# johnnyjana730/MVIN

Measured on AMD Instinct MI355X. Metric: (user,item) pairs scored/sec @ dim=64 hop=2 fan-out=32; % HBM roofline, higher is better.
Workload: dtype f32

## Files before the change

mvin_amd/csrc/mvin_kernels.h:

```cpp
#pragma once
#include <hip/hip_runtime.h>
#include <stdint.h>

#include "../../include/mvin_hip.h"
#include "mvin_common.h"

namespace mvin {

struct GatherAttnArgs {
    int gather;
    int table_bf16;
    const void* table;
    const int32_t* adj_e;
    const int32_t* adj_r;
    const int32_t* node_ids;
    const float* neigh;
    const int32_t* rel_ids;
    const float* rel_score;
    const float* self_vec;
    const float* Wc;
    const float* c_child;
    const float* Wagg;
    const float* bagg;
    float* out;
    float* probs;
    float* s_out;
    float* z_out;
    int64_t T;
    int N, K, D, lpr_log2;
    int tile_rows;
};

struct RippleArgs {
    const void* E;
    int table_bf16;
    const int32_t* score_ids;
    const int32_t* rel_ids;
    const int32_t* value_ids;
    const float* V;
    const float* w;
    float* out;
    int64_t ldo;
    int64_t B;
    int mode, Nm, D, nR, lpr_log2;
};

struct RippleBuildArgs {
    const int64_t* indptr;
    const int32_t* dst;
    const int32_t* rel;
    const int64_t* hist_ptr;
    const int32_t* hist_items;
    int32_t* out;
    int64_t n_user;
    uint64_t seed;
    int P, Nm, n_neighbor;
};

struct KeyAddrArgs {
    const void* E;
    const float* V;
    const float* w;
    const int32_t* mem_h[8];
    const int32_t* mem_r[8];
    const int32_t* mem_t[8];
    float* out;
    int64_t ldo;
    int64_t B;
    int P, Nm, D, nR, lpr_log2;
    uint64_t table_bytes;
    const int32_t* uts;
    const int64_t* users64;
    const int32_t* users32;
    int n_user;
    int n_entity;
};

struct KeyAddrLists {
    const int32_t *h, *r, *t;
};
__device__ __forceinline__ KeyAddrLists key_addr_lists(const KeyAddrArgs& a, int64_t b, int hop) {
    if (a.uts) {
        int64_t u = a.users64 ? a.users64[b] : (int64_t)a.users32[b];
        u = u < 0 ? 0 : (u >= a.n_user ? a.n_user - 1 : u);
        const int32_t* base = a.uts + ((u * (a.P > 0 ? a.P : 1) + hop) * 3) * (int64_t)a.Nm;
        return {base, base + a.Nm, base + 2 * a.Nm};
    }
    const int64_t o = b * a.Nm;
    return {a.mem_h[hop] + o, hop < a.P ? a.mem_r[hop] + o : nullptr, hop < a.P ? a.mem_t[hop] + o : nullptr};
}

struct KeyAddrGroupedArgs {
    const void* E;
    const float* R;
    const float* w;
    const int32_t* uts;
    const int32_t* seg_user;
    const int32_t* seg_ptr;
    const int32_t* nseg_dev;
    const int32_t* pair_index;
    const int64_t* items64;
    const int32_t* items32;
    float* out;
    int64_t ldo;
    int nseg, P, Nm, D, nR, NRL;
    int n_entity;
    int dbg;
    const int32_t* records;
    const float* ER;
    const float* hs;
};

struct KaFlashArgs {
    const float* E;
    const float* ER;
    const float* hs;
    const int32_t* records;
    const int32_t* seg_user;
    const int32_t* seg_ptr;
    const int32_t* nseg_dev;
    const int32_t* pair_index;
    const int64_t* items64;
    const int32_t* items32;
    const float* TW;
    const float* bmlp;
    float* user_o;
    int32_t* slot_seg;
    int32_t* counter;
    int nslots;
    int P, Nm, nR, n_entity;
    int64_t B;
};

struct KaRecLayout {
    int NmP, rows, maxtiles, o_cnt, o_off, o_trel, o_bidx, o_head, o_tail, o_hr, len;
};

struct TailArgs {
    const void* E;
    const int64_t* items64;
    const int32_t* items32;
    const float* q;
    const float* user_o;
    const float* nagg0;
    const float* nagg1;
    const float* W0;
    const float* b0;
    const float* A0;
    const float* a0;
    const float* A1;
    const float* a1;
    const float* Wmix;
    const float* bmix;
    float* item_emb;
    float* scores;
    float* sig;
    int64_t B;
    int table_bf16;
    int n_entity;
    int dbg;
};

struct EntityAggArgs {
    const float* tabS;
    const float* tabG;
    const float* selfS;
    const float* selfG;
    const int32_t* adj_e;
    const int32_t* adj_r;
    const float* t0;
    float* outS;
    float* outG;
    int n_entity, K, nR;
    uint64_t table_bytes, adj_bytes;
    int D;
};

struct TailFoldArgs {
    const float* M0;
    const int64_t* items64;
    const int32_t* items32;
    const float* q;
    const float* user_o;
    const float* out0;
    const float* z2;
    const float* Wqm;
    const float* A1;
    const float* a1;
    const float* Wmix;
    const float* bm;
    float* item_emb;
    float* scores;
    float* sig;
    int64_t B;
    int n_entity;
};

struct GatherMixArgs {
    const void* table;
    const int32_t* adj_e;
    const int32_t* adj_r;
    const int32_t* node_ids;
    const float* rel_score;
    const float* rowbias;
    float* out;
    int64_t nodes;
    int npg, K, D, lpr_log2, relu, table_bf16;
};

struct FusedL2Args {
    const void* table;
    const int32_t* adj_e;
    const int32_t* adj_r;
    const int32_t* parent_ids;
    const float* t0;
    const float* t1;
    const float* W1;
    const float* W2;
    const float* q;
    const float* b1;
    const float* b2;
    const float* A0;
    const float* a0;
    float* nagg0;
    float* nagg1;
    float* probs_parent;
    float* probs_child;
    int64_t P;
    uint64_t table_bytes;
    uint64_t adj_bytes;
    int parents_per_pair, K, nR, lpn_log2;
    int pid_stride;
    unsigned max_id;
    int dbg;
    const int32_t* order;
    float* agg;
    int fold;
    int prj;
};

__device__ __forceinline__ int fused_parent_id(const FusedL2Args& a, int64_t i) {
    const unsigned v = (unsigned)a.parent_ids[i * a.pid_stride];
    return (int)(v < a.max_id ? v : a.max_id);
}

struct EltArgs {
    int mode;
    int64_t n;
    float* x;
    float* y;
    float* z;
    float* w;
    float* accum;
    float alpha, beta, beta1, beta2, eps;
    int D, N;
};

struct WgradArgs {
    mvin_linear_args lin;
    const float* dY;
    int64_t ldy, dy_zstride;
    const float* mask;
    int64_t ldm, mask_zstride;
    float* dW;
    int64_t dw_zstride;
    float* db;
    int64_t db_zstride;
    int IB;
};

struct AggBwdArgs {
    int gather;
    const float* table;
    const int32_t* adj_e;
    const int32_t* adj_r;
    const int32_t* node_ids;
    const float* child;
    const int32_t* rel_ids;
    const float* probs;
    const float* rel_score;
    int skip_zero;
    const float* dvec;
    float* dtable;
    float* dchild;
    float* dT;
    int64_t T;
    int K, D, nR, lpr_log2;
};

struct KeyAddrBwdArgs {
    KeyAddrArgs f;
    const float* dout;
    float* dE;
    float* dV;
    float* dw;
    float l2;
    const float* Rk;
    const void* items;
    int items64;
    int dw_rep;
    int dv_lds;
    float* reg_accum;
};

hipError_t launch_eltwise(const EltArgs& a, hipStream_t st);
hipError_t launch_l2_adam_multi(const mvin_param_seg* segs, int nseg, int64_t total, float* g, float* mo, float* vo,
                                float* accum, int apply_adam, float lr_t, const float* lr_dev, float b1, float b2,
                                float eps, hipStream_t st);
hipError_t launch_l2_adam_multi_guarded(const mvin_param_seg* segs, int nseg, int64_t total, float* g, float* mo, float* vo,
                                        float* accum, int apply_adam, const mvin_guard_state* guard, float b1, float b2,
                                        float eps, hipStream_t st);
hipError_t launch_grad_guard(const mvin_param_seg* segs, int nseg, int64_t total, const float* g,
                             const mvin_guard_item* items, int nitems, mvin_guard_partial* partials,
                             const float* lr_table, int lr_table_len, mvin_guard_state* state, int grid_cap,
                             hipStream_t st);
hipError_t launch_scatter_add_rows(float* dtable, const int32_t* ids, int ids64, const float* x, int64_t rows, int D,
                                   float alpha, hipStream_t st);
hipError_t launch_linear_wgrad(WgradArgs a, hipStream_t st);
hipError_t launch_linear_wgrad_multi(const WgradArgs* probs, int n, hipStream_t st);
hipError_t launch_agg_bwd(const AggBwdArgs& a, hipStream_t st);
hipError_t launch_rel_score_bwd(const float* rel, const float* urh_w, const float* dT, int nR, int D, float* drel,
                                float* durh, hipStream_t st);
hipError_t launch_key_addr_bwd(const KeyAddrBwdArgs& a, hipStream_t st);

inline int lpr_log2_for(int D) {
    int l = 0;
    while ((4 << l) < D) ++l;
    return l;
}

hipError_t launch_expand(const int32_t* adj_e, const int32_t* adj_r, const int64_t* items64,
                         const int32_t* items32, int B, int K, int levels, int n_entity,
                         int32_t* ent_out, int32_t* rel_out, hipStream_t st);
hipError_t launch_rel_score(const float* rel, const float* urh_w, int nR, int D, float* t,
                            hipStream_t st);
hipError_t launch_linear(const mvin_linear_args& a, hipStream_t st);
bool linear_mfma_supported(const mvin_linear_args& a);
hipError_t launch_linear_mfma(const mvin_linear_args& a, hipStream_t st);
hipError_t launch_gather_attn(const GatherAttnArgs& a, hipStream_t st);
hipError_t launch_ripple(const RippleArgs& a, hipStream_t st);
hipError_t launch_sample_adjacency(const int64_t* indptr, const int32_t* dst, const int32_t* rel, int n_entity,
                                   int K, uint64_t seed, int32_t* adj_e, int32_t* adj_r, hipStream_t st);
hipError_t launch_ripple_build(const RippleBuildArgs& a, hipStream_t st);
int key_addr_nj(int Nm, int D);
bool key_addr_grouped_supported(int D, int P, int Nm, int nR);
hipError_t launch_key_addr_grouped(const KeyAddrGroupedArgs& a, int table_bf16, hipStream_t st);
bool key_addr_wave16_supported(int D, int P, int Nm, int nR);
bool key_addr_wave16_applies(const KeyAddrGroupedArgs& a);
hipError_t launch_key_addr_wave16(const KeyAddrGroupedArgs& a, int table_bf16, hipStream_t st);
bool key_addr_dense_supported(int D, int P, int Nm, int nR);
hipError_t launch_key_addr_dense(const KeyAddrGroupedArgs& a, int table_bf16, hipStream_t st);
KaRecLayout ka_rec_layout(int P, int Nm, int nR);
hipError_t launch_user_records(const int32_t* uts, int n_user, int P, int Nm, int nR, int n_entity, int32_t* out, hipStream_t st);
bool key_addr_static_supported(int D, int P, int Nm, int nR);
bool key_addr_static_applies(const KeyAddrGroupedArgs& a, int table_bf16);
hipError_t launch_key_addr_static(const KeyAddrGroupedArgs& a, hipStream_t st);
bool key_addr_flash_supported(int D, int P, int Nm, int nR, int n_entity);
size_t key_addr_flash_ws_elems(int64_t B, int nseg_bound);
hipError_t launch_key_addr_flash(const KaFlashArgs& a, int nseg_bound, bool has_set, int32_t* sched_ws, hipStream_t st);
hipError_t kas_read_trace(long long* host_dst, size_t n);
hipError_t kaf_read_trace(long long* host_dst, size_t n);
hipError_t fold_read_trace(long long* host_dst, size_t n);
hipError_t launch_key_addr(const KeyAddrArgs& a, int table_bf16, hipStream_t st);
bool key_addr_stream_supported(const KeyAddrArgs& a, int table_bf16);
hipError_t launch_key_addr_stream(const KeyAddrArgs& a, int table_bf16, hipStream_t st);
hipError_t launch_move_rows(void* table, const int32_t* ids, int64_t n, int row_bytes, void* rows, bool scatter,
                            hipStream_t st);
hipError_t launch_shard_space_ids(const void* ids, bool is64, int64_t n, int world, int n_local, void* out, hipStream_t st);
hipError_t launch_row_softmax(const float* x, int64_t rows, int n, float* out, hipStream_t st);
hipError_t launch_mix_urv(const float* neigh, const float* rel, const float* user, const float* logits, int64_t nodes, int N, int K,
                          int D, float* out, float* probs, hipStream_t st);
hipError_t launch_gather_mix(const GatherMixArgs& a, hipStream_t st);
struct ScoreSmallArgs {
    const void* E;
    const int32_t* adj_e;
    const int32_t* adj_r;
    const float* R;
    const float* w_h;
    const float* Wu;
    const float* bu;
    const float* t0;
    const float* t1;
    const float *W0, *b0, *W1, *b1, *W2, *b2;
    const float *A0, *a0, *A1, *a1, *Wmix, *bmix;
    const int64_t* items;
    const int32_t* mem_h[4];
    const int32_t* mem_r[4];
    const int32_t* mem_t[4];
    const int32_t* uts;
    const int64_t* users;
    float* user_o;
    float* item_emb;
    float* scores;
    float* sig;
    int64_t B;
    int G;
    int K, P, Nm, nR, n_entity, n_user, enc, table_bf16;
    int depth1;
    int dbg;
    uint64_t table_bytes;
    uint64_t adj_bytes;
};
bool score_small_supported(int D, int K, int P, int Nm, int nR);
int score_small_group(int D, int K, int P, int Nm, int nR, int has_hset, int64_t B);
hipError_t launch_score_small(ScoreSmallArgs a, int D, hipStream_t st);
hipError_t small_read_trace(long long* host_dst, size_t n);

bool l2_tail_supported(int D);
hipError_t launch_l2_tail(const TailArgs& a, int D, hipStream_t st);
bool l2_tail_flash_applies(const TailArgs& a, int D);
hipError_t launch_l2_tail_flash(const TailArgs& a, hipStream_t st);
bool fused_l2_supported(int D, int K);
hipError_t launch_gather_attn_l2(const FusedL2Args& a, int D, int table_bf16, hipStream_t st);
bool fused_split_supported(int D, int K);
bool fused_split_applies(const FusedL2Args& a, int D);
hipError_t launch_gather_probe_l2(const void* table, const int32_t* ids1, const int32_t* ids2, int64_t n_parents, int K,
                                  int D, int table_bf16, float* sums, hipStream_t st);
hipError_t launch_group_pairs(const int64_t* u64, const int32_t* u32, int64_t B, int n_user, int32_t* count, int32_t* offs,
                              int32_t* rank, int32_t* seg_user, int32_t* seg_ptr, int32_t* nseg, int32_t* pair_index, hipStream_t st);
hipError_t launch_count_ids(const int32_t* ids, int64_t n, int nbins, float* out, hipStream_t st);
bool fused_d32_supported(int D, int K);
bool fused_d32_applies(const FusedL2Args& a, int D);
bool topk_rows_supported(int k);
hipError_t launch_topk_rows(const float* scores, int64_t rows, int64_t n, int64_t ld, const int32_t* cand_ids, int64_t col_offset,
                            const int64_t* excl_ptr, const int32_t* excl_ids, const int32_t* carry_ids, const float* carry_vals, int k,
                            int32_t* out_ids, float* out_vals, hipStream_t st);
hipError_t launch_rank_positives(const float* scores, int64_t rows, int64_t n, int64_t ld, const int32_t* cand_ids, int64_t col_offset,
                                 const int64_t* excl_ptr, const int32_t* excl_ids, const int64_t* pos_ptr, const int32_t* pos_ids,
                                 int32_t* out_counts, float* out_vals, int32_t* out_eligible, hipStream_t st);
int64_t ctr_counts_ws_bytes(int64_t n_seg, int64_t seg_len);
hipError_t launch_ctr_counts(const float* scores, const int32_t* labels, int64_t n_seg, int64_t seg_len, int64_t ld, void* ws,
                             int64_t* out, hipStream_t st);
bool sample_negatives_supported(int n_item);
hipError_t launch_sample_negatives(const int64_t* excl_ptr, const int32_t* excl_ids, const int32_t* counts, const int64_t* out_ptr,
                                   int n_user, int n_item, const uint32_t* alias_tab, const uint32_t* mask_bits, uint64_t seed,
                                   uint64_t round, int32_t* out, int64_t* status,
                                   hipStream_t st);
hipError_t launch_rank_head(const float* user_o, const float* item_emb, const float* valid, int64_t n_groups, int G, int D, int mode,
                            float scale, float* scores, float* dscore, float* du, float* di, float* loss_accum, int64_t* counts,
                            hipStream_t st);
hipError_t launch_select_negatives(const float* scores, const int64_t* items, const float* valid, const int64_t* group_key,
                                   int64_t n_groups, int Gp, int n_neg, int shortlist, uint64_t seed, uint64_t round,
                                   int64_t* out_items, float* out_valid, float* out_scores, int64_t* counts,
                                   hipStream_t st);
int64_t kg_explore_ws_bytes(int n_entity, int64_t M);
hipError_t launch_kg_field(const int64_t* eptr, const int32_t* edst, const int32_t* erel, int n_entity, int64_t M,
                           const int32_t* seeds, int64_t n_seed, int hops, void* ws, uint32_t* field_bits, int64_t* out_counts,
                           hipStream_t st);
hipError_t launch_kg_explore(const int64_t* eptr, const int32_t* edst, const int32_t* erel, int n_entity, int64_t M,
                             const int32_t* adj_entity, const int32_t* adj_relation, int K, const int32_t* seeds, int64_t n_seed,
                             int hops, void* ws, uint32_t* explored_bits, int64_t* out_counts, hipStream_t st);
size_t order_ws_elems(int64_t B);
hipError_t launch_order_by_key(const int64_t* k64, const int32_t* k32, int64_t B, int32_t* ws, int32_t* order, hipStream_t st);
bool fused_wpp_supported(int D, int K);
bool fused_wpp_applies(const FusedL2Args& a, int D);
hipError_t launch_gather_attn_l2_wpp(const FusedL2Args& a, hipStream_t st);
bool fused_agg_supported(int D, int K);
bool fused_fold_supported(int D, int K);
size_t fused_fold_lds_bytes(int D, int nR, int K);
bool fused_agg_applies(const FusedL2Args& a, int D);
hipError_t launch_entity_aggregates(const EntityAggArgs& a, hipStream_t st);
hipError_t launch_fold_prepare(const float* W0, const float* b0, const float* W1, const float* b1, const float* W2, const float* b2, const float* A0,
                               const float* a0, const float* Wmix, const float* bmix, const float* A1, float c, int D, float* blk, hipStream_t st);
hipError_t launch_l2_tail_fold(const TailFoldArgs& a, hipStream_t st);
hipError_t launch_score_l2_folded(const float* agg, const float* M0, const int32_t* adj_e, const int32_t* adj_r, const int32_t* items, int pid_stride,
                                  const float* t1, const float* q, const float* user_o, const float* Wq, const float* bq, const float* Wv,
                                  const float* bv, const float* Wqm, const float* A1, const float* a1, const float* Wm1, const float* Wm2,
                                  const float* bm, float* item_emb, float* scores, float* sig, int64_t B, int K, int D, int nR, int n_entity,
                                  hipStream_t st);
hipError_t launch_gather_attn_l2_agg(const FusedL2Args& a, hipStream_t st);
hipError_t launch_gather_attn_l2_d32(const FusedL2Args& a, int table_bf16, hipStream_t st, bool encoded = false);
bool fused_d16_supported(int D, int K);
bool fused_d16_applies(const FusedL2Args& a, int D);
hipError_t launch_gather_attn_l2_d16(const FusedL2Args& a, int table_bf16, hipStream_t st);
bool fused_l2_split_in_use();
hipError_t launch_gather_attn_l2_split(const FusedL2Args& a, int D, int table_bf16, hipStream_t st);
hipError_t split_read_trace(long long* host_dst, size_t n);
bool fused_packed_supported(int D, int K);
bool key_addr_static_er_ok(int P, int Nm, int nR, int n_entity, bool has_set);
hipError_t launch_transpose_blocks(const float* R, int nR, int D, float* RT, hipStream_t st);
constexpr int kEtMaxJobs = 24;
struct EntityTableJob {
    const float* W;
    float* out;
    int w_nk;
};
hipError_t launch_entity_tables(const float* E, int n_entity, const EntityTableJob* jobs, int njobs, hipStream_t st);
hipError_t launch_entity_dot(const float* E, const float* w, int n, int D, float* out, hipStream_t st);
hipError_t launch_prj_prepare(const float* W1, const float* W2, const float* b1, const float* b2, const float* A0, const float* a0,
                              float c, int D, float* blk, hipStream_t st);
bool fused_packed_applies(const FusedL2Args& a, int D);
hipError_t pack_read_prof(long long* host_dst, size_t n);
hipError_t launch_gather_attn_l2_packed(const FusedL2Args& a, int D, int table_bf16, hipStream_t st);
hipError_t launch_encode_adjacency(const int32_t* adj_e, const int32_t* adj_r, int n_entity, int K, int32_t* cnt,
                                   int32_t* enc_e, int32_t* enc_r, hipStream_t st);
hipError_t ka_read_trace(long long* host_dst, size_t n);

}
```

mvin_amd/csrc/mvin_keyaddr_flash.hip:

```cpp
#include <cstdlib>
#include <type_traits>

#include "mvin_kernels.h"

namespace mvin {

typedef float f32x4 __attribute__((ext_vector_type(4)));

constexpr int kFlashChunk = 64;
constexpr int kFlashWaves = 4;

__global__ void ka_flash_slots_kernel(const int32_t* __restrict__ seg_ptr, const int32_t* __restrict__ nseg_dev, int nseg_bound,
                                      int32_t* __restrict__ slot_seg) {
    const int nseg = nseg_dev ? min(*nseg_dev, nseg_bound) : nseg_bound;
    for (int s = blockIdx.x * blockDim.x + threadIdx.x; s < nseg; s += gridDim.x * blockDim.x) {
        const int p0 = seg_ptr[s], p1 = seg_ptr[s + 1];
        const int first = p0 / kFlashChunk + s;
        const int nch = (p1 - p0 + kFlashChunk - 1) / kFlashChunk;
        for (int c = 0; c < nch; ++c) slot_seg[first + c] = s;
    }
}

#define KAF_FENCE() __builtin_amdgcn_sched_barrier(0)

__device__ float g_kaf_no_bias[64];
__device__ long long g_kaf_trace[64 * 16];

extern __shared__ __attribute__((aligned(16))) int32_t sKafRec[];

template <int NMT, bool HAS_SET, bool PF, bool TRACE = false>
__global__ __launch_bounds__(kFlashWaves * 64, 2) void key_addr_flash_kernel(KaFlashArgs a, KaRecLayout RL) {
    constexpr int D = 64;
    __shared__ f32x4 sUo0[kFlashWaves][4][64];
    const int lane = threadIdx.x & 63, l16 = lane & 15, q16 = lane >> 4;
    f32x4 (*myUo0)[64] = sUo0[threadIdx.x >> 6];
    const int P = a.P, NmP = RL.NmP;
    const unsigned emax = (unsigned)(a.n_entity - 1);
    const float* __restrict__ E = a.E;
    const float* __restrict__ bias = a.bmlp;
    const size_t tw_stride = (size_t)a.n_entity * D;

    struct Rows {
        float4 v[NMT][4];
    };
    auto issue_u = [&](int mt, const int (&hr)[NMT], Rows& R) {
        const f32x4* src = reinterpret_cast<const f32x4*>(a.ER + (size_t)(unsigned)max(hr[mt], 0) * D) + q16;
#pragma unroll
        for (int nt = 0; nt < 4; ++nt) {
            const f32x4 v = src[4 * nt];
            R.v[mt][nt] = make_float4(v[0], v[1], v[2], v[3]);
        }
    };
    auto issue_t = [&](int mt, const float* __restrict__ tab, const int4 (&ids)[NMT], Rows& R) {
        const int id[4] = {ids[mt].x, ids[mt].y, ids[mt].z, ids[mt].w};
#pragma unroll
        for (int i = 0; i < 4; ++i)
            R.v[mt][i] = reinterpret_cast<const float4*>(tab + (size_t)(unsigned)max(id[i], 0) * D)[l16];
    };
    auto reads_tile = [&](bool two, int mt, const Rows& R, const f32x4 (&p0)[NMT], const f32x4 (&p1)[NMT], f32x4 (&u0)[4], f32x4 (&u1)[4]) {
        if (two) {
#pragma unroll
            for (int i = 0; i < 4; ++i) {
                const float t[4] = {R.v[mt][i].x, R.v[mt][i].y, R.v[mt][i].z, R.v[mt][i].w};
#pragma unroll
                for (int nt = 0; nt < 4; ++nt) u0[nt] = __builtin_amdgcn_mfma_f32_16x16x4f32(t[nt], p0[mt][i], u0[nt], 0, 0, 0);
#pragma unroll
                for (int nt = 0; nt < 4; ++nt) u1[nt] = __builtin_amdgcn_mfma_f32_16x16x4f32(t[nt], p1[mt][i], u1[nt], 0, 0, 0);
            }
        } else {
#pragma unroll
            for (int i = 0; i < 4; ++i) {
                const float t[4] = {R.v[mt][i].x, R.v[mt][i].y, R.v[mt][i].z, R.v[mt][i].w};
#pragma unroll
                for (int nt = 0; nt < 4; ++nt) u0[nt] = __builtin_amdgcn_mfma_f32_16x16x4f32(t[nt], p0[mt][i], u0[nt], 0, 0, 0);
            }
        }
    };
    auto softmax = [&](f32x4 (&lg)[NMT], const int4 (&ids)[NMT]) {
        float mx = -INFINITY;
#pragma unroll
        for (int mt = 0; mt < NMT; ++mt) {
            const int id[4] = {ids[mt].x, ids[mt].y, ids[mt].z, ids[mt].w};
#pragma unroll
            for (int i = 0; i < 4; ++i) mx = fmaxf(mx, id[i] >= 0 ? lg[mt][i] : -INFINITY);
        }
        mx = xor32_max(xor16_max(mx));
        float z = 0.f;
#pragma unroll
        for (int mt = 0; mt < NMT; ++mt) {
            const int id[4] = {ids[mt].x, ids[mt].y, ids[mt].z, ids[mt].w};
#pragma unroll
            for (int i = 0; i < 4; ++i) {
                const float x = lean_exp(fminf(lg[mt][i] - mx, 0.f));
                const float e = id[i] >= 0 ? x : 0.f;
                lg[mt][i] = e;
                z += e;
            }
        }
        z = xor32_sum(xor16_sum(z));
        const float inv = 1.f / z;
#pragma unroll
        for (int mt = 0; mt < NMT; ++mt) {
#pragma unroll
            for (int i = 0; i < 4; ++i) lg[mt][i] *= inv;
        }
    };

    int iter = 0;
    auto stamp = [&](int slot) {
        if constexpr (TRACE) {
            if (blockIdx.x == 0 && threadIdx.x == 0 && iter >= 2 && iter < 66) g_kaf_trace[(iter - 2) * 16 + slot] = __builtin_readcyclecounter();
        }
    };
    auto load_item_raw = [&](const int (&orig)[2], unsigned (&item)[2]) {
#pragma unroll
        for (int rt = 0; rt < 2; ++rt)
            item[rt] = a.items64 ? reinterpret_cast<const unsigned*>(a.items64)[2 * (int64_t)orig[rt]] : (unsigned)a.items32[orig[rt]];
    };
    auto load_item = [&](const int (&orig)[2], unsigned (&item)[2]) {
        load_item_raw(orig, item);
#pragma unroll
        for (int rt = 0; rt < 2; ++rt) item[rt] = min(item[rt], emax);
    };

    const int wave = __builtin_amdgcn_readfirstlane((int)(threadIdx.x >> 6));
    const int stride = (int)gridDim.x * kFlashWaves;
    const int recW = (1 + 2 * P) * NmP, ldsT = NmP, ldsHr = NmP + P * NmP;
    const unsigned lds0 = (unsigned)(size_t)(__attribute__((address_space(3))) char*)sKafRec + (unsigned)(wave * 2 * recW * 4);
    const int lorig = kFlashWaves * 2 * recW + wave * 32;
    const unsigned ldsOrig = (unsigned)(size_t)(__attribute__((address_space(3))) char*)sKafRec + (unsigned)(lorig * 4);
    auto la_slots_issue = [&](long long base) -> int {
        const long long kc = base + (long long)stride * (lane + 1);
        return kc < a.nslots ? a.slot_seg[kc] : -1;
    };
    auto la_slots_take = [&](long long base, int sv, int& kN, int& sN) -> bool {
        for (;;) {
            const unsigned long long live = __ballot(sv >= 0);
            if (live) {
                const int j = __ffsll(live) - 1;
                kN = __builtin_amdgcn_readfirstlane((int)(base + (long long)stride * (j + 1)));
                sN = __builtin_amdgcn_readlane(sv, j);
                return true;
            }
            base += 64ll * stride;
            if (base + stride >= a.nslots) return false;
            sv = la_slots_issue(base);
        }
    };
    auto la_seg_issue = [&](int s) -> int {
        const int32_t* src = lane == 0 ? a.seg_user + s : a.seg_ptr + s + (lane - 1);
        return lane < 3 ? *src : 0;
    };
    auto la_seg_take = [&](int v, int k, int s, int& u, int& cbeg, int& cend) {
        u = __builtin_amdgcn_readlane(v, 0);
        const int p0 = __builtin_amdgcn_readlane(v, 1), p1 = __builtin_amdgcn_readlane(v, 2);
        cbeg = p0 + (k - (p0 / kFlashChunk + s)) * kFlashChunk;
        cend = min(p1, cbeg + kFlashChunk);
    };
    auto la_rec_issue = [&](int u, int cbeg, int cend, int par) {
        const char* src = reinterpret_cast<const char*>(a.records + (size_t)u * RL.len);
        const unsigned dst = lds0 + (unsigned)(par * recW * 4);
        for (int j0 = 0; j0 < recW; j0 += 64) {
            const int i = j0 + lane;
            if (i < recW) {
                const int voff = 4 * (i < NmP ? RL.o_head + i : RL.o_tail + (i - NmP));
                unsigned keep;
                asm volatile("s_nop 4\n\ts_mov_b32 %0, m0\n\ts_mov_b32 m0, %3\n\ts_nop 0\n\tglobal_load_lds_dword %1, %2\n\ts_mov_b32 m0, %0"
                             : "=&s"(keep)
                             : "v"(voff), "s"(src), "s"(dst + 4u * (unsigned)j0)
                             : "memory");
            }
        }
        if (lane < 32) {
            const int voff = 4 * min(lane, cend - 1 - cbeg);
            unsigned keep;
            asm volatile("s_nop 4\n\ts_mov_b32 %0, m0\n\ts_mov_b32 m0, %3\n\ts_nop 0\n\tglobal_load_lds_dword %1, %2\n\ts_mov_b32 m0, %0"
                         : "=&s"(keep)
                         : "v"(voff), "s"(a.pair_index + cbeg), "s"(ldsOrig)
                         : "memory");
        }
    };
    auto la_orig = [&](int (&orig)[2]) {
#pragma unroll
        for (int rt = 0; rt < 2; ++rt) orig[rt] = sKafRec[lorig + 16 * rt + l16];
    };
    bool nHave = false;
    int nK = 0, nS = 0, nU = 0, nCbeg = 0, nCend = 0;
    int par = 0;
    int laSlots = 0, laSeg = 0;
    unsigned itemP[2] = {0, 0};
    if constexpr (PF) {
        const long long base = (long long)((int)blockIdx.x * kFlashWaves + wave) - stride;
        nHave = la_slots_take(base, la_slots_issue(base), nK, nS);
        if (nHave) {
            la_seg_take(la_seg_issue(nS), nK, nS, nU, nCbeg, nCend);
            la_rec_issue(nU, nCbeg, nCend, par);
            asm volatile("s_waitcnt vmcnt(0)" ::: "memory");
            int o[2];
            la_orig(o);
            load_item_raw(o, itemP);
        }
    }
    for (;; ++iter) {
        stamp(0);
        int k = 0, u = 0, cbeg = 0, cend = 0;
        if constexpr (PF) {
            if (!nHave) break;
            k = nK, u = nU, cbeg = nCbeg, cend = nCend;
            asm volatile("s_waitcnt vmcnt(0)" ::: "memory");
        } else {
            if (lane == 0) k = atomicAdd(a.counter, 1) + 1;
            k = __builtin_amdgcn_readfirstlane(k);
            if (k >= a.nslots) break;
            const int s = __builtin_amdgcn_readfirstlane(a.slot_seg[k]);
            if (s < 0) continue;
            u = __builtin_amdgcn_readfirstlane(a.seg_user[s]);
            const int p0 = __builtin_amdgcn_readfirstlane(a.seg_ptr[s]), p1 = __builtin_amdgcn_readfirstlane(a.seg_ptr[s + 1]);
            cbeg = p0 + (k - (p0 / kFlashChunk + s)) * kFlashChunk;
            cend = min(p1, cbeg + kFlashChunk);
        }
        const int32_t* __restrict__ rec = a.records + (size_t)u * RL.len;
        const int lrec = (wave * 2 + par) * recW;
        stamp(1);
        auto load_hr = [&](int hop, int (&hr)[NMT]) {
#pragma unroll
            for (int mt = 0; mt < NMT; ++mt) {
                if constexpr (PF) hr[mt] = sKafRec[lrec + ldsHr + hop * NmP + 16 * mt + l16];
                else hr[mt] = rec[RL.o_hr + hop * NmP + 16 * mt + l16];
            }
        };
        auto load_tid = [&](int hop, int4 (&tid)[NMT]) {
#pragma unroll
            for (int mt = 0; mt < NMT; ++mt) {
                if constexpr (PF) tid[mt] = *reinterpret_cast<const int4*>(&sKafRec[lrec + ldsT + hop * NmP + 16 * mt + 4 * q16]);
                else tid[mt] = *reinterpret_cast<const int4*>(rec + RL.o_tail + hop * NmP + 16 * mt + 4 * q16);
            }
        };
        auto la_step_slots = [&]() {
            nHave = la_slots_take(k, laSlots, nK, nS);
            if (nHave) laSeg = la_seg_issue(nS);
        };
        auto la_step_seg = [&]() {
            if (nHave) {
                la_seg_take(laSeg, nK, nS, nU, nCbeg, nCend);
                la_rec_issue(nU, nCbeg, nCend, par ^ 1);
            }
        };
        auto la_step_items = [&](bool rows_since) {
            if (nHave) {
                if (!rows_since) asm volatile("s_waitcnt vmcnt(0)" ::: "memory");
                int o[2];
                la_orig(o);
                load_item_raw(o, itemP);
            }
        };
        auto load_orig = [&](int t0, int (&orig)[2], bool (&valid)[2]) {
#pragma unroll
            for (int rt = 0; rt < 2; ++rt) {
                const int p = t0 + 16 * rt + l16;
                valid[rt] = p < cend;
                orig[rt] = a.pair_index[min(p, cend - 1)];
            }
        };
        auto load_be = [&](const unsigned (&item)[2], float4 (&bE)[2][4]) {
#pragma unroll
            for (int rt = 0; rt < 2; ++rt) {
#pragma unroll
                for (int nt = 0; nt < 4; ++nt) bE[rt][nt] = reinterpret_cast<const float4*>(E + (size_t)item[rt] * D)[4 * nt + q16];
            }
        };

        int orig[2], origN[2];
        bool valid[2], validN[2];
        unsigned item[2];
        float4 bE[2][4];
        int hrC[NMT], hrN[NMT];
        int4 tidC[NMT];
        Rows R;
        if constexpr (PF) {
#pragma unroll
            for (int rt = 0; rt < 2; ++rt) item[rt] = min(itemP[rt], emax), valid[rt] = cbeg + 16 * rt + l16 < cend;
            la_orig(orig);
        } else {
            load_orig(cbeg, orig, valid);
        }
        load_hr(0, hrC);
        load_tid(0, tidC);
        load_orig(cbeg + 32, origN, validN);
        f32x4 uo0[4];
#pragma unroll
        for (int r = 0; r < 4; ++r) {
            const float4 b = reinterpret_cast<const float4*>(bias)[4 * q16 + r];
            uo0[0][r] = b.x, uo0[1][r] = b.y, uo0[2][r] = b.z, uo0[3][r] = b.w;
        }
        if constexpr (HAS_SET) {
            int4 hid[NMT];
            f32x4 ph[NMT];
#pragma unroll
            for (int mt = 0; mt < NMT; ++mt) {
                if constexpr (PF) hid[mt] = *reinterpret_cast<const int4*>(&sKafRec[lrec + 16 * mt + 4 * q16]);
                else hid[mt] = *reinterpret_cast<const int4*>(rec + RL.o_head + 16 * mt + 4 * q16);
            }
#pragma unroll
            for (int mt = 0; mt < NMT; ++mt) issue_t(mt, a.TW, hid, R);
            KAF_FENCE();
            stamp(11);
            if constexpr (PF) laSlots = la_slots_issue(k);
#pragma unroll
            for (int mt = 0; mt < NMT; ++mt) {
                const int id[4] = {hid[mt].x, hid[mt].y, hid[mt].z, hid[mt].w};
#pragma unroll
                for (int i = 0; i < 4; ++i) ph[mt][i] = a.hs[max(id[i], 0)];
            }
            if constexpr (!PF) load_item(orig, item);
            KAF_FENCE();
            stamp(12);
            if constexpr (PF) {
                la_step_slots();
                KAF_FENCE();
            }
            softmax(ph, hid);
            KAF_FENCE();
            stamp(13);
            f32x4 unused[4];
#pragma unroll
            for (int mt = 0; mt < NMT; ++mt) {
                reads_tile(false, mt, R, ph, ph, uo0, unused);
                KAF_FENCE();
                issue_u(mt, hrC, R);
                KAF_FENCE();
            }
            stamp(14);
        } else {
            if constexpr (!PF) load_item(orig, item);
#pragma unroll
            for (int mt = 0; mt < NMT; ++mt) issue_u(mt, hrC, R);
            if constexpr (PF) laSlots = la_slots_issue(k);
        }
        load_be(item, bE);
        if constexpr (PF && !HAS_SET) {
            KAF_FENCE();
            la_step_slots();
        }
#pragma unroll
        for (int nt = 0; nt < 4; ++nt) myUo0[nt][lane] = uo0[nt];
        KAF_FENCE();
        stamp(2);

        const int ntile = (cend - cbeg + 31) >> 5;
        int t0 = cbeg;
        int stage = 0;
        const int stage_items = min(2, 2 * ntile * P - 1);
        auto la_stage = [&]() {
            if constexpr (PF) {
                if (stage == 0) la_step_seg();
                if (stage == stage_items) la_step_items(stage_items == 2);
                ++stage;
                KAF_FENCE();
            }
        };
        auto run_tile = [&](const bool two, const bool more) {
            f32x4 uo[2][4];
#pragma unroll
            for (int rt = 0; rt < 2; ++rt) {
#pragma unroll
                for (int nt = 0; nt < 4; ++nt) uo[rt][nt] = myUo0[nt][lane];
            }
            unsigned itemN[2];
            if (more) load_item(origN, itemN);
            for (int hop = 0; hop < P; ++hop) {
                const bool last_hop = hop + 1 == P;
                const bool next_stage = !last_hop || more;
                const int hopN = last_hop ? 0 : hop + 1;
                const float* __restrict__ tw = a.TW + (size_t)(hop + (HAS_SET ? 1 : 0)) * tw_stride;
                if (next_stage) load_hr(hopN, hrN);
                KAF_FENCE();
                if (t0 == cbeg && hop < 3) stamp(3 + 4 * hop);
                f32x4 lg[2][NMT];
#pragma unroll
                for (int mt = 0; mt < NMT; ++mt) {
                    lg[0][mt] = f32x4{0.f, 0.f, 0.f, 0.f};
                    lg[1][mt] = f32x4{0.f, 0.f, 0.f, 0.f};
                    if (two) {
#pragma unroll
                        for (int nt = 0; nt < 4; ++nt) {
                            const float av[4] = {R.v[mt][nt].x, R.v[mt][nt].y, R.v[mt][nt].z, R.v[mt][nt].w};
                            const float e0[4] = {bE[0][nt].x, bE[0][nt].y, bE[0][nt].z, bE[0][nt].w};
                            const float e1[4] = {bE[1][nt].x, bE[1][nt].y, bE[1][nt].z, bE[1][nt].w};
#pragma unroll
                            for (int i = 0; i < 4; ++i) {
                                lg[0][mt] = __builtin_amdgcn_mfma_f32_16x16x4f32(av[i], e0[i], lg[0][mt], 0, 0, 0);
                                lg[1][mt] = __builtin_amdgcn_mfma_f32_16x16x4f32(av[i], e1[i], lg[1][mt], 0, 0, 0);
                            }
                        }
                    } else {
#pragma unroll
                        for (int nt = 0; nt < 4; ++nt) {
                            const float av[4] = {R.v[mt][nt].x, R.v[mt][nt].y, R.v[mt][nt].z, R.v[mt][nt].w};
                            const float e0[4] = {bE[0][nt].x, bE[0][nt].y, bE[0][nt].z, bE[0][nt].w};
#pragma unroll
                            for (int i = 0; i < 4; ++i) lg[0][mt] = __builtin_amdgcn_mfma_f32_16x16x4f32(av[i], e0[i], lg[0][mt], 0, 0, 0);
                        }
                    }
                    KAF_FENCE();
                    issue_t(mt, tw, tidC, R);
                    KAF_FENCE();
                }
                if (last_hop && more) load_be(itemN, bE);
                KAF_FENCE();
                if (t0 == cbeg && hop < 3) stamp(4 + 4 * hop);
                la_stage();
                softmax(lg[0], tidC);
                if (two) softmax(lg[1], tidC);
                KAF_FENCE();
                if (t0 == cbeg && hop < 3) stamp(5 + 4 * hop);
#pragma unroll
                for (int mt = 0; mt < NMT; ++mt) {
                    reads_tile(two, mt, R, lg[0], lg[1], uo[0], uo[1]);
                    KAF_FENCE();
                    if (next_stage) issue_u(mt, hrN, R);
                    KAF_FENCE();
                }
                if (next_stage) load_tid(hopN, tidC);
                if (t0 == cbeg && hop < 3) stamp(6 + 4 * hop);
                la_stage();
            }
#pragma unroll
            for (int rt = 0; rt < 2; ++rt) {
                if (valid[rt] && (rt == 0 || two)) {
#pragma unroll
                    for (int r = 0; r < 4; ++r)
                        *reinterpret_cast<float4*>(a.user_o + (size_t)orig[rt] * D + 16 * q16 + 4 * r) =
                            make_float4(uo[rt][0][r], uo[rt][1][r], uo[rt][2][r], uo[rt][3][r]);
                }
            }
        };
        for (int tile = 0; tile < ntile; ++tile, t0 += 32) {
            const bool more = tile + 1 < ntile;
            run_tile(cend - t0 > 16, more);
#pragma unroll
            for (int rt = 0; rt < 2; ++rt) orig[rt] = origN[rt], valid[rt] = validN[rt];
        }
        stamp(15);
        par ^= 1;
    }
}

hipError_t kaf_read_trace(long long* host_dst, size_t n) {
    const size_t have = sizeof(g_kaf_trace) / sizeof(long long);
    return hipMemcpyFromSymbol(host_dst, HIP_SYMBOL(g_kaf_trace), (n < have ? n : have) * sizeof(long long));
}
#undef KAF_FENCE

bool key_addr_flash_supported(int D, int P, int Nm, int nR, int n_entity) {
    if (D != 64 || P < 1 || P > 8 || Nm < 1 || Nm > 64) return false;
    const KaRecLayout RL = ka_rec_layout(P, Nm, nR);
    if (RL.len == 0) return false;
    return (long long)nR * n_entity < (1ll << 31);
}

size_t key_addr_flash_ws_elems(int64_t B, int nseg_bound) { return (size_t)(B / kFlashChunk + nseg_bound + 1) + 1; }

static int env_int(const char* name, int dflt) {
    const char* v = getenv(name);
    return v && *v ? atoi(v) : dflt;
}

template <int NMT>
static hipError_t launch_flash_n(const KaFlashArgs& a, const KaRecLayout& RL, bool has_set, hipStream_t st) {
    static const bool prefetch = env_int("MVIN_KAF_PREFETCH", 1) != 0;
    static const int grid_cap = env_int("MVIN_KAF_GRID", 0);
    auto k = prefetch ? (has_set ? key_addr_flash_kernel<NMT, true, true> : key_addr_flash_kernel<NMT, false, true>)
                      : (has_set ? key_addr_flash_kernel<NMT, true, false> : key_addr_flash_kernel<NMT, false, false>);
    if constexpr (NMT == 4) {
        static const bool trace = getenv("MVIN_KAF_TRACE") != nullptr;
        if (trace && has_set) k = prefetch ? key_addr_flash_kernel<4, true, true, true> : key_addr_flash_kernel<4, true, false, true>;
    }
    const size_t lds = prefetch ? (size_t)kFlashWaves * (2 * (1 + 2 * a.P) * RL.NmP + 32) * sizeof(int32_t) : 0;
    static thread_local int per_cu[2][9] = {};
    int& pc = per_cu[has_set ? 1 : 0][a.P];
    if (pc == 0) {
        int v = 0;
        if (hipOccupancyMaxActiveBlocksPerMultiprocessor(&v, reinterpret_cast<const void*>(k), kFlashWaves * 64, lds) != hipSuccess || v < 1) v = 2;
        pc = v > 8 ? 8 : v;
    }
    const int64_t want = ((int64_t)a.nslots + kFlashWaves - 1) / kFlashWaves;
    int grid = (int)(want < 256 * (int64_t)pc ? want : 256 * (int64_t)pc);
    if (grid_cap > 0 && grid > grid_cap) grid = grid_cap;
    k<<<grid, kFlashWaves * 64, lds, st>>>(a, RL);
    return hipGetLastError();
}

hipError_t launch_key_addr_flash(const KaFlashArgs& a_, int nseg_bound, bool has_set, int32_t* sched_ws, hipStream_t st) {
    KaFlashArgs a = a_;
    const KaRecLayout RL = ka_rec_layout(a.P, a.Nm, a.nR);
    if (RL.len == 0 || !sched_ws) return hipErrorInvalidValue;
    if (!a.bmlp) {
        void* zeros = nullptr;
        if (hipError_t e = hipGetSymbolAddress(&zeros, HIP_SYMBOL(g_kaf_no_bias)); e != hipSuccess) return e;
        a.bmlp = static_cast<const float*>(zeros);
    }
    a.nslots = (int)(a.B / kFlashChunk + nseg_bound + 1);
    a.slot_seg = sched_ws;
    a.counter = sched_ws + a.nslots;
    hipError_t e = hipMemsetAsync(sched_ws, 0xFF, ((size_t)a.nslots + 1) * sizeof(int32_t), st);
    if (e != hipSuccess) return e;
    {
        const int blocks = nseg_bound < 256 * 64 ? (nseg_bound + 255) / 256 : 64;
        ka_flash_slots_kernel<<<blocks > 0 ? blocks : 1, 256, 0, st>>>(a.seg_ptr, a.nseg_dev, nseg_bound, sched_ws);
        e = hipGetLastError();
        if (e != hipSuccess) return e;
    }
    switch (RL.NmP / 16) {
        case 1: return launch_flash_n<1>(a, RL, has_set, st);
        case 2: return launch_flash_n<2>(a, RL, has_set, st);
        case 3: return launch_flash_n<3>(a, RL, has_set, st);
        case 4: return launch_flash_n<4>(a, RL, has_set, st);
        default: return hipErrorInvalidValue;
    }
}

}
```

Measured before the change: 550.4 million.

## Replace sparse slot map with compacted live-chunk list for flash scheduling

The slots kernel now builds a dense list of live (segment, chunk-start) entries with a wave prefix scan and an atomic append. The old version wrote a sparse slot→segment map that waves had to scan with ballots to skip empty slots. The flash kernel walks this compacted list with a static stride by default, with an optional dynamic atomic-ticket mode behind an env var. This removes the large 0xFF memset and the empty-slot skipping, at the cost of an extra atomic pass. Per-wave trace instrumentation is also added.

```diff
diff --git a/mvin_amd/csrc/mvin_kernels.h b/mvin_amd/csrc/mvin_kernels.h
--- a/mvin_amd/csrc/mvin_kernels.h
+++ b/mvin_amd/csrc/mvin_kernels.h
@@ -125,7 +125,7 @@
     const float* TW;
     const float* bmlp;
     float* user_o;
-    int32_t* slot_seg;
+    const int32_t* live;
     int32_t* counter;
     int nslots;
     int P, Nm, nR, n_entity;
diff --git a/mvin_amd/csrc/mvin_keyaddr_flash.hip b/mvin_amd/csrc/mvin_keyaddr_flash.hip
--- a/mvin_amd/csrc/mvin_keyaddr_flash.hip
+++ b/mvin_amd/csrc/mvin_keyaddr_flash.hip
@@ -9,15 +9,32 @@
 
 constexpr int kFlashChunk = 64;
 constexpr int kFlashWaves = 4;
-
-__global__ void ka_flash_slots_kernel(const int32_t* __restrict__ seg_ptr, const int32_t* __restrict__ nseg_dev, int nseg_bound,
-                                      int32_t* __restrict__ slot_seg) {
+constexpr bool kFlashDrawDynamicDefault = false;
+
+__global__ void ka_flash_slots_kernel(const int32_t* __restrict__ seg_ptr, const int32_t* __restrict__ nseg_dev, int nseg_bound, int cap,
+                                      int32_t* __restrict__ live) {
     const int nseg = nseg_dev ? min(*nseg_dev, nseg_bound) : nseg_bound;
-    for (int s = blockIdx.x * blockDim.x + threadIdx.x; s < nseg; s += gridDim.x * blockDim.x) {
-        const int p0 = seg_ptr[s], p1 = seg_ptr[s + 1];
-        const int first = p0 / kFlashChunk + s;
-        const int nch = (p1 - p0 + kFlashChunk - 1) / kFlashChunk;
-        for (int c = 0; c < nch; ++c) slot_seg[first + c] = s;
+    const int lane = threadIdx.x & 63;
+    for (int s0 = blockIdx.x * blockDim.x + threadIdx.x - lane; s0 < nseg; s0 += gridDim.x * blockDim.x) {
+        const int s = s0 + lane;
+        int p0 = 0, nch = 0;
+        if (s < nseg) {
+            p0 = seg_ptr[s];
+            nch = max(seg_ptr[s + 1] - p0 + kFlashChunk - 1, 0) / kFlashChunk;
+        }
+        int incl = nch;
+#pragma unroll
+        for (int d = 1; d < 64; d <<= 1) {
+            const int t = __shfl_up(incl, d);
+            if (lane >= d) incl += t;
+        }
+        int base = 0;
+        if (lane == 63 && incl > 0) base = atomicAdd(live, incl);
+        base = __shfl(base, 63) + incl - nch;
+        for (int c = 0; c < nch && base + c < cap; ++c) {
+            live[2 + 2 * (size_t)(base + c)] = s;
+            live[3 + 2 * (size_t)(base + c)] = p0 + c * kFlashChunk;
+        }
     }
 }
 
@@ -25,10 +42,12 @@
 
 __device__ float g_kaf_no_bias[64];
 __device__ long long g_kaf_trace[64 * 16];
+constexpr int kKafTraceWaves = 8192;
+__device__ long long g_kaf_wave_trace[1 + 3 * kKafTraceWaves];
 
 extern __shared__ __attribute__((aligned(16))) int32_t sKafRec[];
 
-template <int NMT, bool HAS_SET, bool PF, bool TRACE = false>
+template <int NMT, bool HAS_SET, bool PF, bool DYN, bool TRACE = false>
 __global__ __launch_bounds__(kFlashWaves * 64, 2) void key_addr_flash_kernel(KaFlashArgs a, KaRecLayout RL) {
     constexpr int D = 64;
     __shared__ f32x4 sUo0[kFlashWaves][4][64];
@@ -107,6 +126,9 @@
     };
 
     int iter = 0;
+    [[maybe_unused]] int walked = 0;
+    [[maybe_unused]] long long t_enter = 0;
+    if constexpr (TRACE) t_enter = wall_clock64();
     auto stamp = [&](int slot) {
         if constexpr (TRACE) {
             if (blockIdx.x == 0 && threadIdx.x == 0 && iter >= 2 && iter < 66) g_kaf_trace[(iter - 2) * 16 + slot] = __builtin_readcyclecounter();
@@ -129,33 +151,26 @@
     const unsigned lds0 = (unsigned)(size_t)(__attribute__((address_space(3))) char*)sKafRec + (unsigned)(wave * 2 * recW * 4);
     const int lorig = kFlashWaves * 2 * recW + wave * 32;
     const unsigned ldsOrig = (unsigned)(size_t)(__attribute__((address_space(3))) char*)sKafRec + (unsigned)(lorig * 4);
-    auto la_slots_issue = [&](long long base) -> int {
-        const long long kc = base + (long long)stride * (lane + 1);
-        return kc < a.nslots ? a.slot_seg[kc] : -1;
-    };
-    auto la_slots_take = [&](long long base, int sv, int& kN, int& sN) -> bool {
-        for (;;) {
-            const unsigned long long live = __ballot(sv >= 0);
-            if (live) {
-                const int j = __ffsll(live) - 1;
-                kN = __builtin_amdgcn_readfirstlane((int)(base + (long long)stride * (j + 1)));
-                sN = __builtin_amdgcn_readlane(sv, j);
-                return true;
-            }
-            base += 64ll * stride;
-            if (base + stride >= a.nslots) return false;
-            sv = la_slots_issue(base);
-        }
-    };
-    auto la_seg_issue = [&](int s) -> int {
-        const int32_t* src = lane == 0 ? a.seg_user + s : a.seg_ptr + s + (lane - 1);
-        return lane < 3 ? *src : 0;
-    };
-    auto la_seg_take = [&](int v, int k, int s, int& u, int& cbeg, int& cend) {
+    const int nlive = min(__builtin_amdgcn_readfirstlane(a.live[0]), a.nslots);
+    auto la_ticket_issue = [&]() -> int {
+        int t = 0;
+        if (lane == 0) t = (int)__builtin_amdgcn_atomic_inc32(reinterpret_cast<unsigned*>(a.counter), 0x7fffffffu, __ATOMIC_RELAXED, "agent");
+        return t;
+    };
+    auto la_ent_issue = [&](int i) -> int {
+        return lane < 2 ? a.live[2 + 2 * (size_t)i + lane] : 0;
+    };
+    auto la_ent_take = [&](int v, int& sg, int& cbeg) {
+        sg = __builtin_amdgcn_readlane(v, 0);
+        cbeg = __builtin_amdgcn_readlane(v, 1);
+    };
+    auto la_seg_issue = [&](int sg) -> int {
+        const int32_t* src = lane == 0 ? a.seg_user + sg : a.seg_ptr + sg + 1;
+        return lane < 2 ? *src : 0;
+    };
+    auto la_seg_take = [&](int v, int cbeg, int& u, int& cend) {
         u = __builtin_amdgcn_readlane(v, 0);
-        const int p0 = __builtin_amdgcn_readlane(v, 1), p1 = __builtin_amdgcn_readlane(v, 2);
-        cbeg = p0 + (k - (p0 / kFlashChunk + s)) * kFlashChunk;
-        cend = min(p1, cbeg + kFlashChunk);
+        cend = min(__builtin_amdgcn_readlane(v, 1), cbeg + kFlashChunk);
     };
     auto la_rec_issue = [&](int u, int cbeg, int cend, int par) {
         const char* src = reinterpret_cast<const char*>(a.records + (size_t)u * RL.len);
@@ -185,15 +200,19 @@
         for (int rt = 0; rt < 2; ++rt) orig[rt] = sKafRec[lorig + 16 * rt + l16];
     };
     bool nHave = false;
-    int nK = 0, nS = 0, nU = 0, nCbeg = 0, nCend = 0;
+    int nI = 0, nS = 0, nU = 0, nCbeg = 0, nCend = 0;
     int par = 0;
-    int laSlots = 0, laSeg = 0;
+    int laEnt = 0, laSeg = 0;
+    [[maybe_unused]] int laTick = 0;
     unsigned itemP[2] = {0, 0};
     if constexpr (PF) {
-        const long long base = (long long)((int)blockIdx.x * kFlashWaves + wave) - stride;
-        nHave = la_slots_take(base, la_slots_issue(base), nK, nS);
+        if constexpr (DYN) nI = __builtin_amdgcn_readfirstlane(la_ticket_issue());
+        else nI = (int)blockIdx.x * kFlashWaves + wave;
+        nHave = nI < nlive;
         if (nHave) {
-            la_seg_take(la_seg_issue(nS), nK, nS, nU, nCbeg, nCend);
+            if constexpr (DYN) laTick = la_ticket_issue();
+            la_ent_take(la_ent_issue(nI), nS, nCbeg);
+            la_seg_take(la_seg_issue(nS), nCbeg, nU, nCend);
             la_rec_issue(nU, nCbeg, nCend, par);
             asm volatile("s_waitcnt vmcnt(0)" ::: "memory");
             int o[2];
@@ -203,21 +222,18 @@
     }
     for (;; ++iter) {
         stamp(0);
-        int k = 0, u = 0, cbeg = 0, cend = 0;
+        int u = 0, cbeg = 0, cend = 0;
         if constexpr (PF) {
             if (!nHave) break;
-            k = nK, u = nU, cbeg = nCbeg, cend = nCend;
+            u = nU, cbeg = nCbeg, cend = nCend;
             asm volatile("s_waitcnt vmcnt(0)" ::: "memory");
         } else {
-            if (lane == 0) k = atomicAdd(a.counter, 1) + 1;
-            k = __builtin_amdgcn_readfirstlane(k);
-            if (k >= a.nslots) break;
-            const int s = __builtin_amdgcn_readfirstlane(a.slot_seg[k]);
-            if (s < 0) continue;
-            u = __builtin_amdgcn_readfirstlane(a.seg_user[s]);
-            const int p0 = __builtin_amdgcn_readfirstlane(a.seg_ptr[s]), p1 = __builtin_amdgcn_readfirstlane(a.seg_ptr[s + 1]);
-            cbeg = p0 + (k - (p0 / kFlashChunk + s)) * kFlashChunk;
-            cend = min(p1, cbeg + kFlashChunk);
+            const int k = __builtin_amdgcn_readfirstlane(la_ticket_issue());
+            if (k >= nlive) break;
+            const int sg = __builtin_amdgcn_readfirstlane(a.live[2 + 2 * (size_t)k]);
+            cbeg = __builtin_amdgcn_readfirstlane(a.live[3 + 2 * (size_t)k]);
+            u = __builtin_amdgcn_readfirstlane(a.seg_user[sg]);
+            cend = min(__builtin_amdgcn_readfirstlane(a.seg_ptr[sg + 1]), cbeg + kFlashChunk);
         }
         const int32_t* __restrict__ rec = a.records + (size_t)u * RL.len;
         const int lrec = (wave * 2 + par) * recW;
@@ -236,13 +252,21 @@
                 else tid[mt] = *reinterpret_cast<const int4*>(rec + RL.o_tail + hop * NmP + 16 * mt + 4 * q16);
             }
         };
-        auto la_step_slots = [&]() {
-            nHave = la_slots_take(k, laSlots, nK, nS);
-            if (nHave) laSeg = la_seg_issue(nS);
+        auto la_step_next = [&]() {
+            if constexpr (DYN) nI = __builtin_amdgcn_readfirstlane(laTick);
+            else nI += stride;
+            nHave = nI < nlive;
+            if (nHave) laEnt = la_ent_issue(nI);
+        };
+        auto la_step_ent = [&]() {
+            if (nHave) {
+                la_ent_take(laEnt, nS, nCbeg);
+                laSeg = la_seg_issue(nS);
+            }
         };
         auto la_step_seg = [&]() {
             if (nHave) {
-                la_seg_take(laSeg, nK, nS, nU, nCbeg, nCend);
+                la_seg_take(laSeg, nCbeg, nU, nCend);
                 la_rec_issue(nU, nCbeg, nCend, par ^ 1);
             }
         };
@@ -252,6 +276,7 @@
                 int o[2];
                 la_orig(o);
                 load_item_raw(o, itemP);
+                if constexpr (DYN) laTick = la_ticket_issue();
             }
         };
         auto load_orig = [&](int t0, int (&orig)[2], bool (&valid)[2]) {
@@ -305,7 +330,7 @@
             for (int mt = 0; mt < NMT; ++mt) issue_t(mt, a.TW, hid, R);
             KAF_FENCE();
             stamp(11);
-            if constexpr (PF) laSlots = la_slots_issue(k);
+            if constexpr (PF) la_step_next();
 #pragma unroll
             for (int mt = 0; mt < NMT; ++mt) {
                 const int id[4] = {hid[mt].x, hid[mt].y, hid[mt].z, hid[mt].w};
@@ -316,7 +341,7 @@
             KAF_FENCE();
             stamp(12);
             if constexpr (PF) {
-                la_step_slots();
+                la_step_ent();
                 KAF_FENCE();
             }
             softmax(ph, hid);
@@ -335,12 +360,12 @@
             if constexpr (!PF) load_item(orig, item);
 #pragma unroll
             for (int mt = 0; mt < NMT; ++mt) issue_u(mt, hrC, R);
-            if constexpr (PF) laSlots = la_slots_issue(k);
+            if constexpr (PF) la_step_next();
         }
         load_be(item, bE);
         if constexpr (PF && !HAS_SET) {
             KAF_FENCE();
-            la_step_slots();
+            la_step_ent();
         }
 #pragma unroll
         for (int nt = 0; nt < 4; ++nt) myUo0[nt][lane] = uo0[nt];
@@ -442,13 +467,25 @@
             for (int rt = 0; rt < 2; ++rt) orig[rt] = origN[rt], valid[rt] = validN[rt];
         }
         stamp(15);
+        if constexpr (TRACE) ++walked;
         par ^= 1;
     }
+    if constexpr (TRACE) {
+        const int w = (int)blockIdx.x * kFlashWaves + wave;
+        if (lane == 0 && w < kKafTraceWaves) {
+            if (w == 0) g_kaf_wave_trace[0] = (long long)gridDim.x * kFlashWaves;
+            g_kaf_wave_trace[1 + 3 * w] = t_enter;
+            g_kaf_wave_trace[2 + 3 * w] = wall_clock64();
+            g_kaf_wave_trace[3 + 3 * w] = walked;
+        }
+    }
 }
 
 hipError_t kaf_read_trace(long long* host_dst, size_t n) {
-    const size_t have = sizeof(g_kaf_trace) / sizeof(long long);
-    return hipMemcpyFromSymbol(host_dst, HIP_SYMBOL(g_kaf_trace), (n < have ? n : have) * sizeof(long long));
+    const size_t have = sizeof(g_kaf_trace) / sizeof(long long), more = sizeof(g_kaf_wave_trace) / sizeof(long long);
+    if (hipError_t e = hipMemcpyFromSymbol(host_dst, HIP_SYMBOL(g_kaf_trace), (n < have ? n : have) * sizeof(long long)); e != hipSuccess || n <= have)
+        return e;
+    return hipMemcpyFromSymbol(host_dst + have, HIP_SYMBOL(g_kaf_wave_trace), (n - have < more ? n - have : more) * sizeof(long long));
 }
 #undef KAF_FENCE
 
@@ -459,7 +496,12 @@
     return (long long)nR * n_entity < (1ll << 31);
 }
 
-size_t key_addr_flash_ws_elems(int64_t B, int nseg_bound) { return (size_t)(B / kFlashChunk + nseg_bound + 1) + 1; }
+static int64_t flash_slots_bound(int64_t B, int nseg_bound) {
+    const int64_t n = B / kFlashChunk + nseg_bound;
+    return n < B ? n : B;
+}
+
+size_t key_addr_flash_ws_elems(int64_t B, int nseg_bound) { return 2 + 2 * (size_t)flash_slots_bound(B, nseg_bound); }
 
 static int env_int(const char* name, int dflt) {
     const char* v = getenv(name);
@@ -470,11 +512,18 @@
 static hipError_t launch_flash_n(const KaFlashArgs& a, const KaRecLayout& RL, bool has_set, hipStream_t st) {
     static const bool prefetch = env_int("MVIN_KAF_PREFETCH", 1) != 0;
     static const int grid_cap = env_int("MVIN_KAF_GRID", 0);
-    auto k = prefetch ? (has_set ? key_addr_flash_kernel<NMT, true, true> : key_addr_flash_kernel<NMT, false, true>)
-                      : (has_set ? key_addr_flash_kernel<NMT, true, false> : key_addr_flash_kernel<NMT, false, false>);
+    static const bool dynamic = [] {
+        const char* v = getenv("MVIN_KAF_DRAW");
+        return v && *v ? v[0] == 'd' : kFlashDrawDynamicDefault;
+    }();
+    auto k = !prefetch ? (has_set ? key_addr_flash_kernel<NMT, true, false, true> : key_addr_flash_kernel<NMT, false, false, true>)
+             : dynamic ? (has_set ? key_addr_flash_kernel<NMT, true, true, true> : key_addr_flash_kernel<NMT, false, true, true>)
+                       : (has_set ? key_addr_flash_kernel<NMT, true, true, false> : key_addr_flash_kernel<NMT, false, true, false>);
     if constexpr (NMT == 4) {
         static const bool trace = getenv("MVIN_KAF_TRACE") != nullptr;
-        if (trace && has_set) k = prefetch ? key_addr_flash_kernel<4, true, true, true> : key_addr_flash_kernel<4, true, false, true>;
+        if (trace && has_set)
+            k = !prefetch ? key_addr_flash_kernel<4, true, false, true, true>
+                          : dynamic ? key_addr_flash_kernel<4, true, true, true, true> : key_addr_flash_kernel<4, true, true, false, true>;
     }
     const size_t lds = prefetch ? (size_t)kFlashWaves * (2 * (1 + 2 * a.P) * RL.NmP + 32) * sizeof(int32_t) : 0;
     static thread_local int per_cu[2][9] = {};
@@ -500,14 +549,14 @@
         if (hipError_t e = hipGetSymbolAddress(&zeros, HIP_SYMBOL(g_kaf_no_bias)); e != hipSuccess) return e;
         a.bmlp = static_cast<const float*>(zeros);
     }
-    a.nslots = (int)(a.B / kFlashChunk + nseg_bound + 1);
-    a.slot_seg = sched_ws;
-    a.counter = sched_ws + a.nslots;
-    hipError_t e = hipMemsetAsync(sched_ws, 0xFF, ((size_t)a.nslots + 1) * sizeof(int32_t), st);
+    a.nslots = (int)flash_slots_bound(a.B, nseg_bound);
+    a.live = sched_ws;
+    a.counter = sched_ws + 1;
+    hipError_t e = hipMemsetAsync(sched_ws, 0, 2 * sizeof(int32_t), st);
     if (e != hipSuccess) return e;
     {
         const int blocks = nseg_bound < 256 * 64 ? (nseg_bound + 255) / 256 : 64;
-        ka_flash_slots_kernel<<<blocks > 0 ? blocks : 1, 256, 0, st>>>(a.seg_ptr, a.nseg_dev, nseg_bound, sched_ws);
+        ka_flash_slots_kernel<<<blocks > 0 ? blocks : 1, 256, 0, st>>>(a.seg_ptr, a.nseg_dev, nseg_bound, a.nslots, sched_ws);
         e = hipGetLastError();
         if (e != hipSuccess) return e;
     }
```

After: 554.7 million (median of 6 runs). No clear change (+0.8%).
